# BrandonHanx/TextReID

Measured on AMD Instinct MI355X. Metric: image-text pairs/sec (train), CLIP-RN50 + BiGRU MoCo step, bs128/GPU, higher is better.
Workload: dtype f32; 1 GPU; configs[1]: CLIP-RN50 + GRU, bs128/GPU, 384x128 images, 64-token captions, MoCo queue 8192, fp32, 1xMI355X; random-init weights, synthetic inputs resident in HBM; global_batch=128, parallelism=dp1, optimizer=Adam (fused multi-tensor), step_launch=eager launches, four streams (chosen by the probe over the recorded step)

## Files before the change

include/textreid_hip.h:

```cpp
#ifndef TEXTREID_HIP_H
#define TEXTREID_HIP_H

#include <stdint.h>

#ifdef __cplusplus
extern "C" {
#endif
#if defined(__GNUC__) || defined(__clang__)
#pragma GCC visibility push(default)
#endif

#define TRID_OK 0
#define TRID_E_INVALID (-1)
#define TRID_E_UNSUPPORTED (-2)

#define TRID_VERSION 100

int trid_version(void);
const char* trid_arch(void);
const char* trid_last_error_string(void);

enum {
    TRID_A_KC = 0,
    TRID_A_MC = 1,
// ... 164 lines not shown
                           void* stream);
int trid_bn_bwd_apply_f32(const float* g, const float* y, const float* act, const float* mean,
                          const float* invstd, const float* scale, const float* shift, const float* dgamma,
                          const float* dbeta, int mask_mode, int pooled, int B, int H, int W, int C, float* dy,
                          float* dres, float* amax, void* stream);
int trid_bn_bwd_reduce_bound_f32(const float* g, const float* y, const float* act, const float* mean,
                                 const float* invstd, const float* scale, const float* shift, int mask_mode, int pooled,
                                 int B, int H, int W, int C, float* dgamma, float* dbeta, float* ws, float* bound,
                                 void* stream);
int trid_bn_bwd_reduce_g_f32(const void* g, int g_fmt, const void* y, int y_fmt, const float* act, const float* mean,
                             const float* invstd, const float* scale, const float* shift, int mask_mode,
                             int pooled, int B, int H, int W, int C, float* dgamma, float* dbeta, float* ws,
                             void* stream);
int trid_bn_bwd_apply_p16_f32(const void* g, int g_fmt, const void* y, int y_fmt, const float* act, const float* mean, const float* invstd,
                              const float* scale, const float* shift, const float* dgamma, const float* dbeta,
                              int mask_mode, int pooled, int B, int H, int W, int C, void* dy, int fmt, void* dres,
                              const float* bound, void* stream);

int trid_bn_bwd_dual_reduce_bound_f32(const float* g, const uint64_t* relu_bits, const float* y1, const float* y2, const float* mean1,
                                      const float* invstd1, const float* scale1, const float* mean2, const float* invstd2,
                                      const float* scale2, long long M, int C, float* dgamma1, float* dgamma2, float* dbeta,
                                      float* dbeta2, float* ws, float* bound1, float* bound2, void* stream);
int trid_bn_bwd_dual_apply_p16_f32(const float* g, const uint64_t* relu_bits, const float* y1, const float* y2, const float* mean1,
                                   const float* invstd1, const float* scale1, const float* mean2, const float* invstd2,
                                   const float* scale2, const float* dgamma1, const float* dgamma2, const float* dbeta, long long M,
                                   int C, void* dy1, void* dy2, const float* bound1, const float* bound2, void* stream);

int trid_attnpool_tokens_f32(const float* x, const float* pos, float* tok, int B, int T, int C, int ldt,
                             void* stream);
int trid_attnpool_tokens_fmt_f32(const void* x, int x_fmt, const float* x_amax, const float* pos, float* tok, int B, int T,
                                 int C, int ldt, void* stream);
int trid_attnpool_tokens_bwd_f32(const float* dtok, float* dx, float* dpos, int B, int T, int C, int ldt,
                                 void* stream);
int trid_softmax_rows_f32(float* s, long long rows, int n, int ld, void* stream);
int trid_softmax_rows_bwd_f32(const float* p, const float* dp, float* ds, long long rows, int n, int ld,
                              void* stream);
int trid_colsum_f32(const float* x, float* out, long long M, int N, long long ld, int accumulate, void* stream);

int trid_embedding_gather_f32(const float* table, const int64_t* tokens, float* x, int B, int L, int ldtok, int E,
                              long long vocab, void* stream);
int trid_embedding_bwd_f32(const float* dX, const int64_t* tokens, int B, int L, int ldtok, int E, float* dtable,
                           long long vocab, long long padding_idx, void* stream);
int trid_gru_cell_fwd_f32(const float* gi, const float* gh, float* h, const int64_t* lengths, float* gates,
                          float* hprev, float* maxv, int32_t* argt, int s, int Lmax, int L, int B, int Hd,
                          long long gates_dstride, long long hprev_dstride, void* stream);
int trid_gru_max_init_f32(float* maxv, int32_t* argt, const int64_t* lengths, int Lmax, const int64_t* lmax_dev, int B,
                          int Hd, void* stream);
int trid_gru_cell_bwd_f32(const float* dout, const int32_t* argt, const float* gates, const float* hprev,
                          const int64_t* lengths, float* dh, float* dGi, float* dgh, int s, int Lmax, int L,
                          int B, int Hd, long long gates_dstride, long long hprev_dstride, long long dgh_dstride,
                          void* stream);

long long trid_gru_whh_image_bytes(int H);
int trid_gru_step_workgroups(int B, int H);
int trid_gru_pack_whh_f16(const float* w_hh, const float* w_amax, void* img_fwd, void* img_bwd, int H, void* stream);
int trid_gru_step_fwd_f32(const void* img_fwd, const float* w_amax, const void* hp_in, void* hp_out, float* h,
                          const float* gi, const int64_t* lengths, float* gates, float* hprev, float* maxv,
                          int32_t* argt, int s, int Lmax, int L, int B, int Bp, int H, long long gates_dstride,
                          long long hprev_dstride, void* stream);
int trid_gru_step_bwd_f32(const void* img_bwd, const float* w_amax, const float* dgh_in, const float* amax_in,
                          float* amax_out, const float* dout, const int32_t* argt, const float* gates,
                          const float* hprev, const int64_t* lengths, float* dh, float* dGi, float* dgh_out, int s,
                          int Lmax, int L, int B, int H, long long gates_dstride, long long hprev_dstride,
                          long long dgh_dstride, void* stream);

int trid_gru_step_seq_fwd_f32(const void* img_fwd, const float* w_amax, const void* hp_in, void* hp_out, float* h,
// ... 133 lines not shown
```

textreid_amd/backbones/m_resnet.py:

```python

import logging
import math
import os
from collections import OrderedDict

import torch
from torch import nn

from .. import ops


class Bottleneck(nn.Module):
    expansion = 4

    def __init__(self, inplanes, planes, stride=1):
        super().__init__()
        self.conv1 = nn.Conv2d(inplanes, planes, 1, bias=False)
        self.bn1 = nn.BatchNorm2d(planes)
        self.conv2 = nn.Conv2d(planes, planes, 3, padding=1, bias=False)
        self.bn2 = nn.BatchNorm2d(planes)
        self.avgpool = nn.AvgPool2d(stride) if stride > 1 else nn.Identity()
        self.conv3 = nn.Conv2d(planes, planes * 4, 1, bias=False)
        self.bn3 = nn.BatchNorm2d(planes * 4)
        self.relu = nn.ReLU(inplace=True)
# ... 28 lines not shown
        self.v_proj = nn.Linear(embed_dim, embed_dim)
        self.c_proj = nn.Linear(embed_dim, output_dim or embed_dim)
        self.num_heads = num_heads

    def forward(self, x):
        raise RuntimeError("AttentionPool2d is a parameter holder; call ModifiedResNet.forward")


def _w3x3(conv):
    w = conv.weight
    N, C = w.shape[0], w.shape[1]
    return w.permute(0, 2, 3, 1).contiguous().reshape(N, 9 * C)


def _g3x3(dw, N, C):
    return dw.view(N, 3, 3, C).permute(0, 3, 1, 2)


def _bn_coeffs(bn, partials, M, training, counters=None):
    if training:
        st = ops.bn_finalize(partials, M, bn.weight, bn.bias, bn.running_mean, bn.running_var)
        if counters is None:
            bn.num_batches_tracked += 1
        else:
            counters.append(bn.num_batches_tracked)
        return st
    return ops.bn_eval_coeffs(bn.weight, bn.bias, bn.running_mean, bn.running_var)


import os as _os
_SERIAL_WGRAD = "1" in (_os.environ.get("TRID_SERIAL_WGRAD", "0"), _os.environ.get("TRID_SERIAL", "0"))
_SERIAL_ATTN_WGRAD = _os.environ.get("TRID_SERIAL_ATTN_WGRAD", "0") == "1"
_EARLY_WPT = _os.environ.get("TRID_EARLY_WPT", "1") != "0"
_BATCH_WGRAD = int(_os.environ.get("TRID_WGRAD_BATCH", "1"))


class _WgradStream:

    def __init__(self, device):
        self.main = torch.cuda.current_stream(device)
        self.side = _WgradStream._streams.setdefault(device, torch.cuda.Stream(device=device))
        self.side.wait_stream(self.main)
        self.pending = []
        self.blocks = 0

    _streams = {}

    def run(self, fn, *tensors, keep=()):
        if _SERIAL_WGRAD:
            return fn(*tensors)
        ev = torch.cuda.Event()
        ev.record(self.main)
        self.side.wait_event(ev)
        for t in tensors + tuple(k for k in keep if k is not None):
            t.record_stream(self.side)
        with torch.cuda.stream(self.side):
            out = fn(*tensors)
        out.record_stream(self.main)
        return out

    def defer(self, G, key, fn, tensors, keep=(), post=None):
        if _SERIAL_WGRAD or not _BATCH_WGRAD:
            out = self.run(fn, *tensors, keep=keep)
            G[key] = post(out) if post is not None else out
            return
        self.pending.append((G, key, fn, tensors, keep, post))
# ... 647 lines not shown
            if not stem16:
                x = ops.p16_pack(x, ax, fmt)
            for blk in self.blocks():
                x, rec = block_forward_p16(blk, x, WP, images.device, training, save, nbt, masks)
                if save:
                    S["blocks"].append(rec)
                if taps is not None:
                    taps[names[id(blk)]] = x.unpack()
            if save:
                S["p16"] = fmt
        else:
            for blk in self.blocks():
                x, ax, rec = block_forward(blk, x, ax, ar, training, save, nbt, masks)
                if save:
                    S["blocks"].append(rec)
                if taps is not None:
                    taps[names[id(blk)]] = x
        if nbt:
            torch._foreach_add_(nbt, 1)
        feat, asave = self._attnpool_forward(x, save)
        if save:
            S["attn"] = asave
        return feat, S

    def _attnpool_forward(self, x, save):
        ap = self.attnpool
        B, H, W, C = x.shape
        T = H * W
        T1 = T + 1
        T1p = (T1 + 3) // 4 * 4
        heads = ap.num_heads
        hd = C // heads
        scale = float(hd) ** -0.5
        xd = x.data if isinstance(x, ops.P16) else x
        x_fmt = x.fmt if isinstance(x, ops.P16) else 0
        tok = ops.empty((B, T1p, C), xd)
        ops.call("trid_attnpool_tokens_fmt_f32", ops._p(xd), x_fmt, ops._p(x.amax) if x_fmt == 1 else None, ops._p(ap.positional_embedding),
                 ops._p(tok), B, T, C, T1p, ops.stream())
        x = tok
        q = ops.linear(tok[:, 0], ap.q_proj.weight, ap.q_proj.bias)
        U = ops.empty((B, heads, C), x)
        ops.gemm(q, ap.k_proj.weight, U, B, C, hd, C, C, heads * C, b_mode=ops.B_NC, alpha=scale, batch=heads,
                 strideA=hd, strideB=hd * C, strideC=C)
        P = ops.empty((B, heads, T1p), x)
        ops.gemm(U, tok, P, heads, T1p, C, C, C, T1p, batch=B, strideA=heads * C, strideB=T1p * C, strideC=heads * T1p)
        ops.softmax_rows_(P, T1)
        Z = ops.empty((B, heads, C), x)
        ops.gemm(P, tok, Z, heads, C, T1p, T1p, C, C, b_mode=ops.B_NC, batch=B, strideA=heads * T1p, strideB=T1p * C,
                 strideC=heads * C)
        o = ops.empty((B, C), x)
        ops.gemm(Z, ap.v_proj.weight, o, B, hd, C, heads * C, C, C, batch=heads, strideA=C, strideB=hd * C, strideC=hd,
                 bias=ap.v_proj.bias, strideBias=hd)
        out = ops.linear(o, ap.c_proj.weight, ap.c_proj.bias)
        return out, (((B, H, W, C), tok, q, U, P, Z, o) if save else None)

    def _attnpool_backward(self, asave, gout, G, ws=None):
        ap = self.attnpool
        xshape, tok, q, U, P, Z, o = asave
        B, H, W, C = xshape
        T = H * W
        T1 = T + 1
        T1p = tok.shape[1]
        heads = ap.num_heads
        hd = C // heads
        scale = float(hd) ** -0.5
        Wq, Wk, Wv, Wc = ap.q_proj.weight, ap.k_proj.weight, ap.v_proj.weight, ap.c_proj.weight
        def side(key, fn, *tensors):
            if ws is None or _SERIAL_ATTN_WGRAD:
                G[key] = fn(*tensors)
            else:
                ws.defer(G, key, fn, tensors)

        do = ops.matmul_nn(gout, Wc)
        side(id(Wc), lambda g_, o_: ops.matmul_tn(g_, o_), gout, o)
        side(id(ap.c_proj.bias), lambda g_: ops.colsum(g_), gout)
        side(id(ap.v_proj.bias), lambda d_: ops.colsum(d_), do)

        def dwv(do_, Z_):
            out = torch.empty_like(Wv)
            ops.gemm(do_, Z_, out, hd, C, B, C, heads * C, C, a_mode=ops.A_MC, b_mode=ops.B_NC, batch=heads, strideA=hd,
                     strideB=C, strideC=hd * C)
            return out

        side(id(Wv), dwv, do, Z)
        dZ = ops.empty((B, heads, C), tok)
        ops.gemm(do, Wv, dZ, B, C, hd, C, C, heads * C, b_mode=ops.B_NC, batch=heads, strideA=hd, strideB=hd * C,
                 strideC=C)
        dP = ops.empty((B, heads, T1p), tok)
        ops.gemm(dZ, tok, dP, heads, T1p, C, C, C, T1p, batch=B, strideA=heads * C, strideB=T1p * C,
                 strideC=heads * T1p)
        dS = ops.softmax_rows_bwd(P, dP, T1, out=dP)
        dtok = ops.empty((B, T1p, C), tok)
        ops.gemm(P, dZ, dtok, T1p, C, heads, T1p, C, C, a_mode=ops.A_MC, b_mode=ops.B_NC, batch=B,
                 strideA=heads * T1p, strideB=heads * C, strideC=T1p * C)
        ops.gemm(dS, U, dtok, T1p, C, heads, T1p, C, C, a_mode=ops.A_MC, b_mode=ops.B_NC, batch=B,
                 strideA=heads * T1p, strideB=heads * C, strideC=T1p * C, accumulate=True)
        dU = ops.empty((B, heads, C), tok)
        ops.gemm(dS, tok, dU, heads, C, T1p, T1p, C, C, b_mode=ops.B_NC, batch=B, strideA=heads * T1p,
                 strideB=T1p * C, strideC=heads * C)
        dq = ops.empty((B, C), tok)
        ops.gemm(dU, Wk, dq, B, hd, C, heads * C, C, C, alpha=scale, batch=heads, strideA=C, strideB=hd * C, strideC=hd)
        def dwk(q_, dU_):
            out = torch.empty_like(Wk)
            ops.gemm(q_, dU_, out, hd, C, B, C, heads * C, C, a_mode=ops.A_MC, b_mode=ops.B_NC, alpha=scale, batch=heads,
                     strideA=hd, strideB=C, strideC=hd * C)
            return out

        side(id(Wk), dwk, q, dU)
        G[id(ap.k_proj.bias)] = torch.zeros_like(ap.k_proj.bias)
        ops.matmul_nn(dq, Wq, out=dtok[:, 0], accumulate=True)
        side(id(Wq), lambda dq_, tok_: ops.matmul_tn(dq_, tok_[:, 0]), dq, tok)
        side(id(ap.q_proj.bias), lambda dq_: ops.colsum(dq_), dq)
        dx = ops.empty((B, H, W, C), tok)
        dpos = torch.empty_like(ap.positional_embedding)
        ops.call("trid_attnpool_tokens_bwd_f32", ops._p(dtok), ops._p(dx), ops._p(dpos), B, T, C, T1p, ops.stream())
        G[id(ap.positional_embedding)] = dpos
        if ws is not None:
            ws.flush()
        return dx

    def _run_backward(self, S, gout):
        G = {}
        ws = _WgradStream(gout.device)
        ar = ConvArith(gout.device, S.get("wamax", {}), S.get("prec"))
        g = self._attnpool_backward(S["attn"], gout, G, ws)
        S["attn"] = None
        blocks = list(self.blocks())
        sync = self.grad_sync
        staged = set()

        def stage_ready():
            if sync is None:
                return
            ws.join()
            ps = [p for p in self.parameters() if id(p) in G and id(p) not in staged and G[id(p)] is not None]
            staged.update(id(p) for p in ps)
            sync.stage(ps, [G[id(p)] for p in ps])

        first_of_layer = {id(layer[0]) for layer in (self.layer1, self.layer2, self.layer3, self.layer4)}
        dbg = getattr(self, "_debug_grads", None)
        p16 = S.get("p16", 0)
        WPT = (S.get("WPT") or p16_weights(self, ar.WA, True, p16)) if p16 else None
        if p16 == 2 and ops.BF16_GRADS:
            g = g.to(torch.bfloat16)
        rblocks, rrecs = list(reversed(blocks)), list(reversed(S["blocks"]))
        g_sums = None
        for bi, (blk, rec) in enumerate(zip(rblocks, rrecs)):
            if dbg is not None:
# ... 72 lines not shown
```

textreid_amd/ops.py:

```python

import ctypes
import os
import math

import torch

from . import lib as L
from .lib import GemmDesc, call

A_KC, A_MC, A_CONV = L.TRID_A_KC, L.TRID_A_MC, L.TRID_A_CONV
B_KC, B_NC, B_CONV = L.TRID_B_KC, L.TRID_B_NC, L.TRID_B_CONV

BN_EPS = 1e-5
BN_MOMENTUM = 0.1
STATS_ROWS = 128
GEMM_PRECISION = int(__import__("os").environ.get("TRID_GEMM_PRECISION", "6"))
CONV_PRECISION = int(__import__("os").environ.get("TRID_CONV_PRECISION", "16"))


def conv_precision():
    return CONV_PRECISION if GEMM_PRECISION == 6 else GEMM_PRECISION


_raw_stream = torch._C._cuda_getCurrentRawStream
# ... 1009 lines not shown


def _bn_ws(C, like):
    key = (C, like.device, stream(like.device))
    ws = _ws_cache.get(key)
    if ws is None:
        ws = empty((L.load().trid_bn_bwd_ws_floats(C),), like)
        _ws_cache[key] = ws
    return ws


def bn_bwd(g, y, st, gamma_like, mask_mode, act=None, pooled=False, want_dres=False, amax=None):
    Bi, H, W, C = y.shape
    dg = empty((2, C), y)
    dgamma, dbeta = dg[0], dg[1]
    ws = _bn_ws(C, y)
    call("trid_bn_bwd_reduce_f32", _p(g), _p(y), _p(act), _p(st.mean), _p(st.invstd), _p(st.scale), _p(st.shift),
         mask_mode, 1 if pooled else 0, Bi, H, W, C, _p(dgamma), _p(dbeta), _p(ws), stream())
    dy = torch.empty_like(y)
    dres = torch.empty_like(y) if want_dres else None
    call("trid_bn_bwd_apply_f32", _p(g), _p(y), _p(act), _p(st.mean), _p(st.invstd), _p(st.scale), _p(st.shift),
         _p(dgamma), _p(dbeta), mask_mode, 1 if pooled else 0, Bi, H, W, C, _p(dy), _p(dres), _p(amax), stream())
    return dy, dgamma, dbeta, dres


def colsum(x2d, out=None, accumulate=False):
    M, N = x2d.shape
    if out is None:
        out = empty((N,), x2d)
    call("trid_colsum_f32", _p(x2d), _p(out), M, N, x2d.stride(0), 1 if accumulate else 0, stream())
    return out


def softmax_rows_(s, n):
    rows, ld = s.numel() // s.shape[-1], s.shape[-1]
    call("trid_softmax_rows_f32", _p(s), rows, n, ld, stream())
    return s


def softmax_rows_bwd(p, dp, n, out=None):
    rows, ld = p.numel() // p.shape[-1], p.shape[-1]
    if out is None:
        out = torch.empty_like(p)
    call("trid_softmax_rows_bwd_f32", _p(p), _p(dp), _p(out), rows, n, ld, stream())
    return out


def l2norm_rows(x, eps=1e-12):
    rows, C = x.shape
    y = torch.empty_like(x)
    inv = empty((rows,), x)
    call("trid_l2norm_rows_f32", _p(x), _p(y), _p(inv), rows, C, eps, stream())
    return y, inv


def l2norm_rows_bwd(dy, y, inv, dx=None, accumulate=False):
    rows, C = y.shape
    if dx is None:
        dx = torch.empty_like(y)
    call("trid_l2norm_rows_bwd_f32", _p(dy), _p(y), _p(inv), _p(dx), rows, C, 1 if accumulate else 0, stream())
    return dx


def rowdot(x, y):
    rows, C = x.shape
    out = empty((rows,), x)
# ... 16 lines not shown
```

Measured before the change: 3163 pairs/s.

## Fuse attention-pool token construction into score and weighted-sum kernels

Measured after the change: 3190 pairs/s (median of 6 runs). Within noise of the previous version (+0.8%).

```diff
diff --git a/include/textreid_hip.h b/include/textreid_hip.h
--- a/include/textreid_hip.h
+++ b/include/textreid_hip.h
@@ -220,6 +220,17 @@
                                  int C, int ldt, void* stream);
 int trid_attnpool_tokens_bwd_f32(const float* dtok, float* dx, float* dpos, int B, int T, int C, int ldt,
                                  void* stream);
+int trid_attnpool_fused_ok(int B, int T, int C, int heads, int x_fmt);
+int trid_attnpool_mean_fmt_f32(const void* x, int x_fmt, const float* x_amax, const float* pos, float* tok0, int B, int T,
+                               int C, void* stream);
+int trid_attnpool_scores_fmt_f32(const void* x, int x_fmt, const float* x_amax, const float* tok0, const float* pos,
+                                 const float* A, float* S, int B, int T, int C, int heads, int ldp, void* stream);
+int trid_attnpool_wsum_fmt_f32(const void* x, int x_fmt, const float* x_amax, const float* tok0, const float* pos,
+                               const float* W, float* out, int B, int T, int C, int heads, int ldp, void* stream);
+int trid_attnpool_dtok0_f32(const float* P, const float* dS, const float* dZ, const float* U, float* dtok0, int B, int C,
+                            int heads, int ldp, void* stream);
+int trid_attnpool_dx_f32(const float* P, const float* dS, const float* dZ, const float* U, const float* dtok0, float* dx,
+                         float* dpos, int B, int T, int C, int heads, int ldp, void* stream);
 int trid_softmax_rows_f32(float* s, long long rows, int n, int ld, void* stream);
 int trid_softmax_rows_bwd_f32(const float* p, const float* dp, float* ds, long long rows, int n, int ld,
                               void* stream);
diff --git a/textreid_amd/backbones/m_resnet.py b/textreid_amd/backbones/m_resnet.py
--- a/textreid_amd/backbones/m_resnet.py
+++ b/textreid_amd/backbones/m_resnet.py
@@ -84,6 +84,7 @@
 _SERIAL_WGRAD = "1" in (_os.environ.get("TRID_SERIAL_WGRAD", "0"), _os.environ.get("TRID_SERIAL", "0"))
 _SERIAL_ATTN_WGRAD = _os.environ.get("TRID_SERIAL_ATTN_WGRAD", "0") == "1"
 _EARLY_WPT = _os.environ.get("TRID_EARLY_WPT", "1") != "0"
+_ATTNPOOL_FUSED = _os.environ.get("TRID_ATTNPOOL_FUSED", "1") != "0"
 _BATCH_WGRAD = int(_os.environ.get("TRID_WGRAD_BATCH", "1"))
 
 
@@ -797,35 +798,51 @@
         heads = ap.num_heads
         hd = C // heads
         scale = float(hd) ** -0.5
-        xd = x.data if isinstance(x, ops.P16) else x
-        x_fmt = x.fmt if isinstance(x, ops.P16) else 0
-        tok = ops.empty((B, T1p, C), xd)
-        ops.call("trid_attnpool_tokens_fmt_f32", ops._p(xd), x_fmt, ops._p(x.amax) if x_fmt == 1 else None, ops._p(ap.positional_embedding),
-                 ops._p(tok), B, T, C, T1p, ops.stream())
-        x = tok
-        q = ops.linear(tok[:, 0], ap.q_proj.weight, ap.q_proj.bias)
-        U = ops.empty((B, heads, C), x)
-        ops.gemm(q, ap.k_proj.weight, U, B, C, hd, C, C, heads * C, b_mode=ops.B_NC, alpha=scale, batch=heads,
-                 strideA=hd, strideB=hd * C, strideC=C)
-        P = ops.empty((B, heads, T1p), x)
-        ops.gemm(U, tok, P, heads, T1p, C, C, C, T1p, batch=B, strideA=heads * C, strideB=T1p * C, strideC=heads * T1p)
-        ops.softmax_rows_(P, T1)
-        Z = ops.empty((B, heads, C), x)
-        ops.gemm(P, tok, Z, heads, C, T1p, T1p, C, C, b_mode=ops.B_NC, batch=B, strideA=heads * T1p, strideB=T1p * C,
-                 strideC=heads * C)
+        pos = ap.positional_embedding
+        if _ATTNPOOL_FUSED and ops.attnpool_fused_ok(x, heads):
+            tok0 = ops.attnpool_mean(x, pos)
+            q = ops.linear(tok0, ap.q_proj.weight, ap.q_proj.bias)
+            U = ops.empty((B, heads, C), tok0)
+            ops.gemm(q, ap.k_proj.weight, U, B, C, hd, C, C, heads * C, b_mode=ops.B_NC, alpha=scale, batch=heads,
+                     strideA=hd, strideB=hd * C, strideC=C)
+            P = ops.attnpool_scores(x, tok0, pos, U, ops.empty((B, heads, T1p), tok0))
+            ops.softmax_rows_(P, T1)
+            Z = ops.attnpool_wsum(x, tok0, pos, P)
+            src = (x, tok0)
+            x = tok0
+        else:
+            xd = x.data if isinstance(x, ops.P16) else x
+            x_fmt = x.fmt if isinstance(x, ops.P16) else 0
+            tok = ops.empty((B, T1p, C), xd)
+            ops.call("trid_attnpool_tokens_fmt_f32", ops._p(xd), x_fmt, ops._p(x.amax) if x_fmt == 1 else None, ops._p(pos),
+                     ops._p(tok), B, T, C, T1p, ops.stream())
+            x = tok
+            q = ops.linear(tok[:, 0], ap.q_proj.weight, ap.q_proj.bias)
+            U = ops.empty((B, heads, C), x)
+            ops.gemm(q, ap.k_proj.weight, U, B, C, hd, C, C, heads * C, b_mode=ops.B_NC, alpha=scale, batch=heads,
+                     strideA=hd, strideB=hd * C, strideC=C)
+            P = ops.empty((B, heads, T1p), x)
+            ops.gemm(U, tok, P, heads, T1p, C, C, C, T1p, batch=B, strideA=heads * C, strideB=T1p * C, strideC=heads * T1p)
+            ops.softmax_rows_(P, T1)
+            Z = ops.empty((B, heads, C), x)
+            ops.gemm(P, tok, Z, heads, C, T1p, T1p, C, C, b_mode=ops.B_NC, batch=B, strideA=heads * T1p, strideB=T1p * C,
+                     strideC=heads * C)
+            src = tok
         o = ops.empty((B, C), x)
         ops.gemm(Z, ap.v_proj.weight, o, B, hd, C, heads * C, C, C, batch=heads, strideA=C, strideB=hd * C, strideC=hd,
                  bias=ap.v_proj.bias, strideBias=hd)
         out = ops.linear(o, ap.c_proj.weight, ap.c_proj.bias)
-        return out, (((B, H, W, C), tok, q, U, P, Z, o) if save else None)
+        return out, (((B, H, W, C), src, q, U, P, Z, o) if save else None)
 
     def _attnpool_backward(self, asave, gout, G, ws=None):
         ap = self.attnpool
-        xshape, tok, q, U, P, Z, o = asave
+        xshape, src, q, U, P, Z, o = asave
+        fused = isinstance(src, tuple)
+        tok = src[1] if fused else src
         B, H, W, C = xshape
         T = H * W
         T1 = T + 1
-        T1p = tok.shape[1]
+        T1p = P.shape[2]
         heads = ap.num_heads
         hd = C // heads
         scale = float(hd) ** -0.5
@@ -851,18 +868,24 @@
         dZ = ops.empty((B, heads, C), tok)
         ops.gemm(do, Wv, dZ, B, C, hd, C, C, heads * C, b_mode=ops.B_NC, batch=heads, strideA=hd, strideB=hd * C,
                  strideC=C)
-        dP = ops.empty((B, heads, T1p), tok)
-        ops.gemm(dZ, tok, dP, heads, T1p, C, C, C, T1p, batch=B, strideA=heads * C, strideB=T1p * C,
-                 strideC=heads * T1p)
-        dS = ops.softmax_rows_bwd(P, dP, T1, out=dP)
-        dtok = ops.empty((B, T1p, C), tok)
-        ops.gemm(P, dZ, dtok, T1p, C, heads, T1p, C, C, a_mode=ops.A_MC, b_mode=ops.B_NC, batch=B,
-                 strideA=heads * T1p, strideB=heads * C, strideC=T1p * C)
-        ops.gemm(dS, U, dtok, T1p, C, heads, T1p, C, C, a_mode=ops.A_MC, b_mode=ops.B_NC, batch=B,
-                 strideA=heads * T1p, strideB=heads * C, strideC=T1p * C, accumulate=True)
-        dU = ops.empty((B, heads, C), tok)
-        ops.gemm(dS, tok, dU, heads, C, T1p, T1p, C, C, b_mode=ops.B_NC, batch=B, strideA=heads * T1p,
-                 strideB=T1p * C, strideC=heads * C)
+        pos = ap.positional_embedding
+        if fused:
+            dP = ops.attnpool_scores(src[0], tok, pos, dZ, ops.empty((B, heads, T1p), tok))
+            dS = ops.softmax_rows_bwd(P, dP, T1, out=dP)
+            dU = ops.attnpool_wsum(src[0], tok, pos, dS)
+        else:
+            dP = ops.empty((B, heads, T1p), tok)
+            ops.gemm(dZ, tok, dP, heads, T1p, C, C, C, T1p, batch=B, strideA=heads * C, strideB=T1p * C,
+                     strideC=heads * T1p)
+            dS = ops.softmax_rows_bwd(P, dP, T1, out=dP)
+            dtok = ops.empty((B, T1p, C), tok)
+            ops.gemm(P, dZ, dtok, T1p, C, heads, T1p, C, C, a_mode=ops.A_MC, b_mode=ops.B_NC, batch=B,
+                     strideA=heads * T1p, strideB=heads * C, strideC=T1p * C)
+            ops.gemm(dS, U, dtok, T1p, C, heads, T1p, C, C, a_mode=ops.A_MC, b_mode=ops.B_NC, batch=B,
+                     strideA=heads * T1p, strideB=heads * C, strideC=T1p * C, accumulate=True)
+            dU = ops.empty((B, heads, C), tok)
+            ops.gemm(dS, tok, dU, heads, C, T1p, T1p, C, C, b_mode=ops.B_NC, batch=B, strideA=heads * T1p,
+                     strideB=T1p * C, strideC=heads * C)
         dq = ops.empty((B, C), tok)
         ops.gemm(dU, Wk, dq, B, hd, C, heads * C, C, C, alpha=scale, batch=heads, strideA=C, strideB=hd * C, strideC=hd)
         def dwk(q_, dU_):
@@ -873,12 +896,19 @@
 
         side(id(Wk), dwk, q, dU)
         G[id(ap.k_proj.bias)] = torch.zeros_like(ap.k_proj.bias)
-        ops.matmul_nn(dq, Wq, out=dtok[:, 0], accumulate=True)
-        side(id(Wq), lambda dq_, tok_: ops.matmul_tn(dq_, tok_[:, 0]), dq, tok)
-        side(id(ap.q_proj.bias), lambda dq_: ops.colsum(dq_), dq)
-        dx = ops.empty((B, H, W, C), tok)
-        dpos = torch.empty_like(ap.positional_embedding)
-        ops.call("trid_attnpool_tokens_bwd_f32", ops._p(dtok), ops._p(dx), ops._p(dpos), B, T, C, T1p, ops.stream())
+        dpos = torch.empty_like(pos)
+        if fused:
+            dtok0 = ops.attnpool_dtok0(P, dS, dZ, U)
+            ops.matmul_nn(dq, Wq, out=dtok0, accumulate=True)
+            side(id(Wq), lambda dq_, tok0_: ops.matmul_tn(dq_, tok0_), dq, tok)
+            side(id(ap.q_proj.bias), lambda dq_: ops.colsum(dq_), dq)
+            dx = ops.attnpool_dx(P, dS, dZ, U, dtok0, (B, H, W, C), dpos)
+        else:
+            ops.matmul_nn(dq, Wq, out=dtok[:, 0], accumulate=True)
+            side(id(Wq), lambda dq_, tok_: ops.matmul_tn(dq_, tok_[:, 0]), dq, tok)
+            side(id(ap.q_proj.bias), lambda dq_: ops.colsum(dq_), dq)
+            dx = ops.empty((B, H, W, C), tok)
+            ops.call("trid_attnpool_tokens_bwd_f32", ops._p(dtok), ops._p(dx), ops._p(dpos), B, T, C, T1p, ops.stream())
         G[id(ap.positional_embedding)] = dpos
         if ws is not None:
             ws.flush()
diff --git a/textreid_amd/csrc/attn_pool.hip b/textreid_amd/csrc/attn_pool.hip
--- /dev/null
+++ b/textreid_amd/csrc/attn_pool.hip
@@ -0,0 +1,494 @@
+
+#include "split_common.h"
+
+namespace trid {
+
+typedef float ap16f __attribute__((ext_vector_type(16)));
+
+__device__ __forceinline__ float4 ap_add4(float4 a, float4 b) { return make_float4(a.x + b.x, a.y + b.y, a.z + b.z, a.w + b.w); }
+__device__ __forceinline__ float4 ap_zero4() { return make_float4(0.f, 0.f, 0.f, 0.f); }
+__device__ __forceinline__ int ap_row(int r, int kh) { return (r & 3) + 8 * (r >> 2) + 4 * kh; }
+
+__device__ __forceinline__ void ap_xcd_unit(int id, int inner, int& unit, int& in) {
+    const int per = 8 * inner, grp = id / per, w = id - grp * per;
+    unit = 8 * grp + (w & 7);
+    in = w >> 3;
+}
+static inline unsigned ap_xcd_grid(long long units, int inner) { return (unsigned)((units + 7) / 8 * 8 * inner); }
+
+template <int IFMT>
+__device__ __forceinline__ float4 ap_load_x4(const void* __restrict__ x, long long row, int cq, int CQ, float inv) {
+    if (IFMT == 1) return p16_load4_rc(reinterpret_cast<const uint2*>(x), row, cq, CQ, inv);
+    if (IFMT == 2) return bf16_load4(reinterpret_cast<const uint2*>(x), row * CQ + cq);
+    return reinterpret_cast<const float4*>(x)[row * CQ + cq];
+}
+
+typedef float apf4 __attribute__((ext_vector_type(4)));
+constexpr unsigned AP_OOB = 0x80000000u;
+__device__ __forceinline__ __amdgpu_buffer_rsrc_t ap_rsrc(const void* p, long long bytes) {
+    return __builtin_amdgcn_make_buffer_rsrc((void*)p, 0, (unsigned)bytes, 0x00020000);
+}
+__device__ __forceinline__ float4 ap_bload4(const __amdgpu_buffer_rsrc_t& rs, unsigned off) {
+    const apf4 v = __builtin_bit_cast(apf4, __builtin_amdgcn_raw_buffer_load_b128(rs, off, 0, 0));
+    return make_float4(v.x, v.y, v.z, v.w);
+}
+__device__ __forceinline__ float ap_bload1(const __amdgpu_buffer_rsrc_t& rs, unsigned off) {
+    return __builtin_bit_cast(float, __builtin_amdgcn_raw_buffer_load_b32(rs, off, 0, 0));
+}
+template <int IFMT>
+__device__ __forceinline__ uint4 ap_bload_x4_raw(const __amdgpu_buffer_rsrc_t& rs, unsigned row, int cq, int CQ, bool ok) {
+    if (IFMT == 1) {
+        const unsigned off = ok ? row * (unsigned)CQ * 16u + (unsigned)((cq >> 3) * 16 + (cq & 7)) * 8u : AP_OOB;
+        const uint2 h = __builtin_bit_cast(uint2, __builtin_amdgcn_raw_buffer_load_b64(rs, off, 0, 0));
+        const uint2 l = __builtin_bit_cast(uint2, __builtin_amdgcn_raw_buffer_load_b64(rs, off + 64u, 0, 0));
+        return make_uint4(h.x, h.y, l.x, l.y);
+    }
+    if (IFMT == 2) {
+        const uint2 u = __builtin_bit_cast(uint2, __builtin_amdgcn_raw_buffer_load_b64(rs, ok ? (row * (unsigned)CQ + (unsigned)cq) * 8u : AP_OOB, 0, 0));
+        return make_uint4(u.x, u.y, 0u, 0u);
+    }
+    return __builtin_bit_cast(uint4, __builtin_amdgcn_raw_buffer_load_b128(rs, ok ? (row * (unsigned)CQ + (unsigned)cq) * 16u : AP_OOB, 0, 0));
+}
+template <int IFMT>
+__device__ __forceinline__ float4 ap_decode_x4(uint4 q, float inv) {
+    if (IFMT == 1) {
+        const f16x2 h0 = __builtin_bit_cast(f16x2, q.x), h1 = __builtin_bit_cast(f16x2, q.y);
+        const f16x2 l0 = __builtin_bit_cast(f16x2, q.z), l1 = __builtin_bit_cast(f16x2, q.w);
+        return make_float4(((float)h0.x + (float)l0.x) * inv, ((float)h0.y + (float)l0.y) * inv,
+                           ((float)h1.x + (float)l1.x) * inv, ((float)h1.y + (float)l1.y) * inv);
+    }
+    if (IFMT == 2)
+        return make_float4(__builtin_bit_cast(float, q.x << 16), __builtin_bit_cast(float, q.x & 0xffff0000u),
+                           __builtin_bit_cast(float, q.y << 16), __builtin_bit_cast(float, q.y & 0xffff0000u));
+    return make_float4(__builtin_bit_cast(float, q.x), __builtin_bit_cast(float, q.y), __builtin_bit_cast(float, q.z), __builtin_bit_cast(float, q.w));
+}
+template <int IFMT>
+__device__ __forceinline__ float4 ap_bload_x4(const __amdgpu_buffer_rsrc_t& rs, unsigned row, int cq, int CQ, float inv, bool ok) {
+    return ap_decode_x4<IFMT>(ap_bload_x4_raw<IFMT>(rs, row, cq, CQ, ok), inv);
+}
+__device__ __forceinline__ long long ap_x_bytes(int IFMT, long long rows, int CQ) { return rows * CQ * (IFMT == 2 ? 8 : 16); }
+
+template <int IFMT>
+__global__ __launch_bounds__(256) void attnpool_mean_kernel(const void* __restrict__ x, const float* __restrict__ x_amax,
+                                                            const float4* __restrict__ pos, float4* __restrict__ tok0, int T, int CQ) {
+    __shared__ float4 red[4][64];
+    const int cl = threadIdx.x & 63, tl = threadIdx.x >> 6;
+    const int cq = blockIdx.x * 64 + cl, b = blockIdx.y;
+    const bool live = cq < CQ;
+    const float inv_scale = IFMT == 1 ? 1.f / f16_scale_of(*x_amax) : 1.f;
+    float4 s = ap_zero4();
+    if (live) {
+#pragma unroll 4
+        for (int t = tl; t < T; t += 4) s = ap_add4(s, ap_load_x4<IFMT>(x, (long long)b * T + t, cq, CQ, inv_scale));
+    }
+    red[tl][cl] = s;
+    __syncthreads();
+    if (tl == 0 && live) {
+        const float4 a = red[0][cl], c = red[1][cl], d = red[2][cl], e = red[3][cl];
+        const float inv = 1.f / (float)T;
+        const float4 p0 = pos[cq];
+        tok0[(long long)b * CQ + cq] = make_float4(((a.x + c.x) + (d.x + e.x)) * inv + p0.x, ((a.y + c.y) + (d.y + e.y)) * inv + p0.y,
+                                                  ((a.z + c.z) + (d.z + e.z)) * inv + p0.z, ((a.w + c.w) + (d.w + e.w)) * inv + p0.w);
+    }
+}
+
+constexpr int AP_LD = 132;
+
+template <int IFMT>
+__global__ __launch_bounds__(256) void attnpool_scores_kernel(const void* __restrict__ x, const float* __restrict__ x_amax,
+                                                              const float4* __restrict__ tok0, const float4* __restrict__ pos,
+                                                              const float4* __restrict__ A, float* __restrict__ S, int B, int T,
+                                                              int CQ, int heads, int ldp) {
+    __shared__ float sA[32 * AP_LD];
+    __shared__ float sT[32 * AP_LD];
+    __shared__ float red[4][32][33];
+    const int tid = threadIdx.x, lane = tid & 63, wave = tid >> 6, r = lane & 31, kh = lane >> 5;
+    int b, tile;
+    ap_xcd_unit(blockIdx.x, (T + 31) / 32, b, tile);
+    if (b >= B) return;
+    const int t0 = 1 + tile * 32;
+    const float inv_scale = IFMT == 1 ? 1.f / f16_scale_of(*x_amax) : 1.f;
+    const int lq = tid & 31, lr = tid >> 5;
+    const __amdgpu_buffer_rsrc_t rsX = ap_rsrc(x, ap_x_bytes(IFMT, (long long)B * T, CQ));
+    const __amdgpu_buffer_rsrc_t rsP = ap_rsrc(pos, (long long)(T + 1) * CQ * 16);
+    const __amdgpu_buffer_rsrc_t rsA = ap_rsrc(A, (long long)B * heads * CQ * 16);
+    float4 ra[4], rp[4], rk[4];
+    uint4 rx[4];
+#pragma unroll
+    for (int j = 0; j < 4; ++j) rk[j] = ap_zero4();
+    auto gload = [&](int chunk) {
+        const int cq = chunk * 32 + lq;
+#pragma unroll
+        for (int i = 0; i < 4; ++i) {
+            const int row = lr + 8 * i, t = t0 + row;
+            const bool tok_ok = t <= T;
+            ra[i] = ap_bload4(rsA, row < heads ? (unsigned)((b * heads + row) * CQ + cq) * 16u : AP_OOB);
+            rx[i] = ap_bload_x4_raw<IFMT>(rsX, (unsigned)(b * T + t - 1), cq, CQ, tok_ok);
+            rp[i] = ap_bload4(rsP, tok_ok ? (unsigned)(t * CQ + cq) * 16u : AP_OOB);
+        }
+        if (tile == 0) {
+#pragma unroll
+            for (int j = 0; j < 4; ++j) rk[j] = tok0[(long long)b * CQ + chunk * 32 + 4 * (tid & 7) + j];
+        }
+    };
+    ap16f acc;
+#pragma unroll
+    for (int i = 0; i < 16; ++i) acc[i] = 0.f;
+    float s0 = 0.f;
+    const int nch = CQ / 32;
+    gload(0);
+    for (int ch = 0; ch < nch; ++ch) {
+        __syncthreads();
+#pragma unroll
+        for (int i = 0; i < 4; ++i) {
+            *reinterpret_cast<float4*>(&sA[(lr + 8 * i) * AP_LD + 4 * lq]) = ra[i];
+            *reinterpret_cast<float4*>(&sT[(lr + 8 * i) * AP_LD + 4 * lq]) = ap_add4(ap_decode_x4<IFMT>(rx[i], inv_scale), rp[i]);
+        }
+        __syncthreads();
+        if (tile == 0) {
+            const int h = tid >> 3, part = tid & 7;
+#pragma unroll
+            for (int j = 0; j < 4; ++j) {
+                const float4 u = *reinterpret_cast<const float4*>(&sA[h * AP_LD + 16 * part + 4 * j]);
+                s0 = fmaf(u.w, rk[j].w, fmaf(u.z, rk[j].z, fmaf(u.y, rk[j].y, fmaf(u.x, rk[j].x, s0))));
+            }
+        }
+        if (ch + 1 < nch) gload(ch + 1);
+#pragma unroll
+        for (int g = 0; g < 2; ++g) {
+            const int off = r * AP_LD + 32 * wave + 16 * g + 8 * kh;
+            const float4 a0 = *reinterpret_cast<const float4*>(&sA[off]), a1 = *reinterpret_cast<const float4*>(&sA[off + 4]);
+            const float4 v0 = *reinterpret_cast<const float4*>(&sT[off]), v1 = *reinterpret_cast<const float4*>(&sT[off + 4]);
+            acc = __builtin_amdgcn_mfma_f32_32x32x2f32(a0.x, v0.x, acc, 0, 0, 0);
+            acc = __builtin_amdgcn_mfma_f32_32x32x2f32(a0.y, v0.y, acc, 0, 0, 0);
+            acc = __builtin_amdgcn_mfma_f32_32x32x2f32(a0.z, v0.z, acc, 0, 0, 0);
+            acc = __builtin_amdgcn_mfma_f32_32x32x2f32(a0.w, v0.w, acc, 0, 0, 0);
+            acc = __builtin_amdgcn_mfma_f32_32x32x2f32(a1.x, v1.x, acc, 0, 0, 0);
+            acc = __builtin_amdgcn_mfma_f32_32x32x2f32(a1.y, v1.y, acc, 0, 0, 0);
+            acc = __builtin_amdgcn_mfma_f32_32x32x2f32(a1.z, v1.z, acc, 0, 0, 0);
+            acc = __builtin_amdgcn_mfma_f32_32x32x2f32(a1.w, v1.w, acc, 0, 0, 0);
+        }
+    }
+#pragma unroll
+    for (int i = 0; i < 16; ++i) red[wave][ap_row(i, kh)][r] = acc[i];
+    __syncthreads();
+    for (int idx = tid; idx < 1024; idx += 256) {
+        const int h = idx >> 5, j = idx & 31;
+        const float s = ((red[0][h][j] + red[1][h][j]) + red[2][h][j]) + red[3][h][j];
+        if (h < heads && t0 + j <= T) S[((long long)b * heads + h) * ldp + t0 + j] = s;
+    }
+    if (tile == 0) {
+        s0 += __shfl_xor(s0, 1, 64);
+        s0 += __shfl_xor(s0, 2, 64);
+        s0 += __shfl_xor(s0, 4, 64);
+        if ((tid & 7) == 0 && (tid >> 3) < heads) S[((long long)b * heads + (tid >> 3)) * ldp] = s0;
+    }
+}
+
+struct ApSumFrag {
+    float a[4];
+    float4 v[4];
+};
+
+template <int IFMT>
+__global__ __launch_bounds__(256) void attnpool_wsum_kernel(const void* __restrict__ x, const float* __restrict__ x_amax,
+                                                            const float4* __restrict__ tok0, const float4* __restrict__ pos,
+                                                            const float* __restrict__ Wt, float4* __restrict__ out, int T, int CQ,
+                                                            int heads, int ldp) {
+    __shared__ float smem[3 * 32 * AP_LD];
+    __shared__ float w0[32];
+    float(*red)[32][AP_LD] = reinterpret_cast<float(*)[32][AP_LD]>(smem);
+    const int tid = threadIdx.x, lane = tid & 63, wave = tid >> 6, r = lane & 31, kh = lane >> 5;
+    const int b = blockIdx.y, cq = blockIdx.x * 32 + r;
+    const float inv_scale = IFMT == 1 ? 1.f / f16_scale_of(*x_amax) : 1.f;
+    const __amdgpu_buffer_rsrc_t rsX = ap_rsrc(x, ap_x_bytes(IFMT, (long long)gridDim.y * T, CQ));
+    const __amdgpu_buffer_rsrc_t rsP = ap_rsrc(pos, (long long)(T + 1) * CQ * 16);
+    const int ldw = (T + 1) | 1;
+    {
+        const int n4 = heads * ldp / 4;
+        const __amdgpu_buffer_rsrc_t rsW = ap_rsrc(Wt + (long long)b * heads * ldp, (long long)n4 * 16);
+        for (int base = 0; base < n4; base += 1024) {
+            float4 v[4];
+#pragma unroll
+            for (int k = 0; k < 4; ++k) v[k] = ap_bload4(rsW, base + tid + 256 * k < n4 ? (unsigned)(base + tid + 256 * k) * 16u : AP_OOB);
+#pragma unroll
+            for (int k = 0; k < 4; ++k) {
+                const int f = 4 * (base + tid + 256 * k), h = f / ldp, t = f - h * ldp;
+                if (f < 4 * n4) {
+                    const float e[4] = {v[k].x, v[k].y, v[k].z, v[k].w};
+#pragma unroll
+                    for (int j = 0; j < 4; ++j)
+                        if (t + j <= T) smem[h * ldw + t + j] = e[j];
+                }
+            }
+        }
+        for (int i = heads * ldw + tid; i < 32 * ldw; i += 256) smem[i] = 0.f;
+        if (tid < 32) w0[tid] = tid < heads ? Wt[((long long)b * heads + tid) * ldp] : 0.f;
+    }
+    __syncthreads();
+    const float* Wr = smem + r * ldw;
+    const int npairs = (T + 1) / 2;
+
+    auto load = [&](ApSumFrag& f, int p0) {
+#pragma unroll
+        for (int u = 0; u < 4; ++u) {
+            const int t = 1 + 2 * (p0 + 4 * u) + kh;
+            const bool ok = t <= T;
+            const float w = Wr[ok ? t : T];
+            f.a[u] = ok ? w : 0.f;
+            f.v[u] = ap_add4(ap_bload_x4<IFMT>(rsX, (unsigned)(b * T + t - 1), cq, CQ, inv_scale, ok),
+                             ap_bload4(rsP, ok ? (unsigned)(t * CQ + cq) * 16u : AP_OOB));
+        }
+    };
+    ap16f acc[4];
+#pragma unroll
+    for (int n = 0; n < 4; ++n)
+#pragma unroll
+        for (int i = 0; i < 16; ++i) acc[n][i] = 0.f;
+    auto mma = [&](const ApSumFrag& f) {
+#pragma unroll
+        for (int u = 0; u < 4; ++u) {
+            acc[0] = __builtin_amdgcn_mfma_f32_32x32x2f32(f.a[u], f.v[u].x, acc[0], 0, 0, 0);
+            acc[1] = __builtin_amdgcn_mfma_f32_32x32x2f32(f.a[u], f.v[u].y, acc[1], 0, 0, 0);
+            acc[2] = __builtin_amdgcn_mfma_f32_32x32x2f32(f.a[u], f.v[u].z, acc[2], 0, 0, 0);
+            acc[3] = __builtin_amdgcn_mfma_f32_32x32x2f32(f.a[u], f.v[u].w, acc[3], 0, 0, 0);
+        }
+    };
+    ApSumFrag f0, f1;
+    load(f0, wave);
+    for (int p0 = wave; p0 < npairs; p0 += 32) {
+        load(f1, p0 + 16);
+        mma(f0);
+        load(f0, p0 + 32);
+        mma(f1);
+    }
+    const float4 k0 = tok0[(long long)b * CQ + cq];
+    __syncthreads();
+    if (wave > 0) {
+#pragma unroll
+        for (int i = 0; i < 16; ++i)
+            *reinterpret_cast<float4*>(&red[wave - 1][ap_row(i, kh)][4 * r]) = make_float4(acc[0][i], acc[1][i], acc[2][i], acc[3][i]);
+    }
+    __syncthreads();
+    if (wave == 0) {
+#pragma unroll
+        for (int i = 0; i < 16; ++i) {
+            const int h = ap_row(i, kh);
+            float4 v = make_float4(acc[0][i], acc[1][i], acc[2][i], acc[3][i]);
+            v = ap_add4(v, *reinterpret_cast<const float4*>(&red[0][h][4 * r]));
+            v = ap_add4(v, *reinterpret_cast<const float4*>(&red[1][h][4 * r]));
+            v = ap_add4(v, *reinterpret_cast<const float4*>(&red[2][h][4 * r]));
+            const float w = w0[h];
+            v = make_float4(fmaf(w, k0.x, v.x), fmaf(w, k0.y, v.y), fmaf(w, k0.z, v.z), fmaf(w, k0.w, v.w));
+            if (h < heads) out[((long long)b * heads + h) * CQ + cq] = v;
+        }
+    }
+}
+
+__global__ __launch_bounds__(256) void attnpool_dtok0_kernel(const float* __restrict__ P, const float* __restrict__ dS,
+                                                             const float4* __restrict__ dZ, const float4* __restrict__ U,
+                                                             float4* __restrict__ d0, int CQ, int heads, int ldp) {
+    __shared__ float4 red[4][64];
+    const int cl = threadIdx.x & 63, hl = threadIdx.x >> 6;
+    const int cq = blockIdx.x * 64 + cl;
+    const long long b = blockIdx.y;
+    const bool live = cq < CQ;
+    float4 s = ap_zero4();
+    if (live) {
+#pragma unroll 4
+        for (int h = hl; h < heads; h += 4) {
+            const float p = P[(b * heads + h) * ldp], d = dS[(b * heads + h) * ldp];
+            const float4 z = dZ[(b * heads + h) * CQ + cq], u = U[(b * heads + h) * CQ + cq];
+            s.x = fmaf(d, u.x, fmaf(p, z.x, s.x));
+            s.y = fmaf(d, u.y, fmaf(p, z.y, s.y));
+            s.z = fmaf(d, u.z, fmaf(p, z.z, s.z));
+            s.w = fmaf(d, u.w, fmaf(p, z.w, s.w));
+        }
+    }
+    red[hl][cl] = s;
+    __syncthreads();
+    if (hl == 0 && live) {
+        const float4 a = red[0][cl], c = red[1][cl], d = red[2][cl], e = red[3][cl];
+        d0[b * CQ + cq] = make_float4((a.x + c.x) + (d.x + e.x), (a.y + c.y) + (d.y + e.y), (a.z + c.z) + (d.z + e.z), (a.w + c.w) + (d.w + e.w));
+    }
+}
+
+__global__ __launch_bounds__(256) void attnpool_dx_kernel(const float* __restrict__ P, const float* __restrict__ dS,
+                                                          const float4* __restrict__ dZ, const float4* __restrict__ U,
+                                                          const float4* __restrict__ d0, float4* __restrict__ dx, int B, int T,
+                                                          int CQ, int heads, int ldp) {
+    const int lane = threadIdx.x & 63, wave = threadIdx.x >> 6, r = lane & 31, kh = lane >> 5;
+    const int ncg = (CQ + 127) / 128;
+    int unit, tile;
+    ap_xcd_unit(blockIdx.x, (T + 31) / 32, unit, tile);
+    if (unit >= B * ncg) return;
+    const int cqb = ((unit % ncg) * 4 + wave) * 32;
+    if (cqb >= CQ) return;
+    const int cq = cqb + r;
+    const long long b = unit / ncg;
+    const int t0 = 1 + tile * 32, t = t0 + r;
+    const bool tok_ok = t <= T;
+    const long long nimg = B;
+    const __amdgpu_buffer_rsrc_t rsP = ap_rsrc(P, nimg * heads * ldp * 4), rsD = ap_rsrc(dS, nimg * heads * ldp * 4);
+    const __amdgpu_buffer_rsrc_t rsZ = ap_rsrc(dZ, nimg * heads * CQ * 16), rsU = ap_rsrc(U, nimg * heads * CQ * 16);
+    ap16f acc[4];
+#pragma unroll
+    for (int n = 0; n < 4; ++n)
+#pragma unroll
+        for (int i = 0; i < 16; ++i) acc[n][i] = 0.f;
+    struct Frag {
+        float a1[2], a2[2];
+        float4 zb[2], ub[2];
+    };
+    auto load = [&](Frag& f, int kk) {
+#pragma unroll
+        for (int u = 0; u < 2; ++u) {
+            const int h = 2 * (kk + u) + kh;
+            const bool hok = h < heads;
+            const unsigned row = (unsigned)((int)b * heads + h);
+            const unsigned aoff = (hok && tok_ok) ? (row * (unsigned)ldp + (unsigned)t) * 4u : AP_OOB;
+            const unsigned boff = hok ? (row * (unsigned)CQ + (unsigned)cq) * 16u : AP_OOB;
+            f.a1[u] = ap_bload1(rsP, aoff);
+            f.a2[u] = ap_bload1(rsD, aoff);
+            f.zb[u] = ap_bload4(rsZ, boff);
+            f.ub[u] = ap_bload4(rsU, boff);
+        }
+    };
+    auto mma = [&](const Frag& f) {
+#pragma unroll
+        for (int u = 0; u < 2; ++u) {
+            acc[0] = __builtin_amdgcn_mfma_f32_32x32x2f32(f.a1[u], f.zb[u].x, acc[0], 0, 0, 0);
+            acc[1] = __builtin_amdgcn_mfma_f32_32x32x2f32(f.a1[u], f.zb[u].y, acc[1], 0, 0, 0);
+            acc[2] = __builtin_amdgcn_mfma_f32_32x32x2f32(f.a1[u], f.zb[u].z, acc[2], 0, 0, 0);
+            acc[3] = __builtin_amdgcn_mfma_f32_32x32x2f32(f.a1[u], f.zb[u].w, acc[3], 0, 0, 0);
+            acc[0] = __builtin_amdgcn_mfma_f32_32x32x2f32(f.a2[u], f.ub[u].x, acc[0], 0, 0, 0);
+            acc[1] = __builtin_amdgcn_mfma_f32_32x32x2f32(f.a2[u], f.ub[u].y, acc[1], 0, 0, 0);
+            acc[2] = __builtin_amdgcn_mfma_f32_32x32x2f32(f.a2[u], f.ub[u].z, acc[2], 0, 0, 0);
+            acc[3] = __builtin_amdgcn_mfma_f32_32x32x2f32(f.a2[u], f.ub[u].w, acc[3], 0, 0, 0);
+        }
+    };
+    const int steps = (heads + 1) / 2;
+    Frag f0, f1;
+    load(f0, 0);
+    for (int kk = 0; kk < steps; kk += 4) {
+        load(f1, kk + 2);
+        mma(f0);
+        load(f0, kk + 4);
+        mma(f1);
+    }
+    const float inv = 1.f / (float)T;
+    const float4 m = d0[b * CQ + cq];
+#pragma unroll
+    for (int i = 0; i < 16; ++i) {
+        const int tt = t0 + ap_row(i, kh);
+        if (tt <= T)
+            dx[(b * T + tt - 1) * CQ + cq] = make_float4(acc[0][i] + m.x * inv, acc[1][i] + m.y * inv, acc[2][i] + m.z * inv, acc[3][i] + m.w * inv);
+    }
+}
+
+__global__ __launch_bounds__(256) void attnpool_dpos0_kernel(const float4* __restrict__ d0, float4* __restrict__ dpos, int B, int CQ) {
+    __shared__ float4 red[16][16];
+    const int cl = threadIdx.x & 15, bl = threadIdx.x >> 4;
+    const int cq = blockIdx.x * 16 + cl;
+    float4 s = ap_zero4();
+    if (cq < CQ) {
+#pragma unroll 8
+        for (int b = bl; b < B; b += 16) s = ap_add4(s, d0[(long long)b * CQ + cq]);
+    }
+    red[bl][cl] = s;
+    __syncthreads();
+    if (bl == 0 && cq < CQ) {
+        for (int k = 1; k < 16; ++k) s = ap_add4(s, red[k][cl]);
+        dpos[cq] = s;
+    }
+}
+
+__global__ __launch_bounds__(256) void attnpool_dpos_kernel(const float4* __restrict__ dx, float4* __restrict__ dpos, int B, int T,
+                                                            int CQ) {
+    __shared__ float4 red[4][64];
+    const int cl = threadIdx.x & 63, bl = threadIdx.x >> 6;
+    const long long col = (long long)blockIdx.x * 64 + cl, ncol = (long long)T * CQ;
+    const bool live = col < ncol;
+    float4 s = ap_zero4();
+    if (live) {
+#pragma unroll 4
+        for (int b = bl; b < B; b += 4) s = ap_add4(s, dx[(long long)b * ncol + col]);
+    }
+    red[bl][cl] = s;
+    __syncthreads();
+    if (bl == 0 && live) {
+        const float4 a = red[0][cl], c = red[1][cl], d = red[2][cl], e = red[3][cl];
+        const float inv = 1.f / (float)T;
+        const float4 m = dpos[col % CQ];
+        dpos[CQ + col] = make_float4(((a.x + c.x) + (d.x + e.x)) - m.x * inv, ((a.y + c.y) + (d.y + e.y)) - m.y * inv,
+                                     ((a.z + c.z) + (d.z + e.z)) - m.z * inv, ((a.w + c.w) + (d.w + e.w)) - m.w * inv);
+    }
+}
+
+static bool attnpool_fused_shape_ok(long long B, long long T, long long C, long long heads, int x_fmt) {
+    return B >= 1 && B <= 65535 && T >= 1 && T <= 3 * AP_LD - 2 && B * (T + 4 > 32 ? T + 4 : 32) * C * 4 < (1ll << 31) && C >= 128 && C % 128 == 0 && C <= (1 << 16) && heads >= 1 && heads <= 32 &&
+           x_fmt >= 0 && x_fmt <= 2;
+}
+
+}
+
+using namespace trid;
+
+#define AP_DISPATCH(kernel, grid, ...)                                                                             \
+    do {                                                                                                           \
+        if (x_fmt == 1) hipLaunchKernelGGL(kernel<1>, grid, dim3(256), 0, (hipStream_t)stream, __VA_ARGS__);       \
+        else if (x_fmt == 2) hipLaunchKernelGGL(kernel<2>, grid, dim3(256), 0, (hipStream_t)stream, __VA_ARGS__);  \
+        else hipLaunchKernelGGL(kernel<0>, grid, dim3(256), 0, (hipStream_t)stream, __VA_ARGS__);                  \
+    } while (0)
+
+extern "C" int trid_attnpool_fused_ok(int B, int T, int C, int heads, int x_fmt) {
+    return attnpool_fused_shape_ok(B, T, C, heads, x_fmt) ? 1 : 0;
+}
+
+extern "C" int trid_attnpool_mean_fmt_f32(const void* x, int x_fmt, const float* x_amax, const float* pos, float* tok0, int B, int T,
+                                          int C, void* stream) {
+    TRID_REQUIRE(x && pos && tok0 && (x_fmt != 1 || x_amax) && attnpool_fused_shape_ok(B, T, C, 1, x_fmt), "trid_attnpool_mean_fmt_f32: bad arguments");
+    const int CQ = C / 4;
+    AP_DISPATCH(attnpool_mean_kernel, dim3((unsigned)((CQ + 63) / 64), (unsigned)B), x, x_amax, (const float4*)pos, (float4*)tok0, T, CQ);
+    return check_launch("trid_attnpool_mean_fmt_f32");
+}
+
+extern "C" int trid_attnpool_scores_fmt_f32(const void* x, int x_fmt, const float* x_amax, const float* tok0, const float* pos,
+                                            const float* A, float* S, int B, int T, int C, int heads, int ldp, void* stream) {
+    TRID_REQUIRE(x && tok0 && pos && A && S && (x_fmt != 1 || x_amax) && ldp >= T + 1 && attnpool_fused_shape_ok(B, T, C, heads, x_fmt),
+                 "trid_attnpool_scores_fmt_f32: bad arguments");
+    AP_DISPATCH(attnpool_scores_kernel, dim3(ap_xcd_grid(B, (T + 31) / 32)), x, x_amax, (const float4*)tok0, (const float4*)pos,
+                (const float4*)A, S, B, T, C / 4, heads, ldp);
+    return check_launch("trid_attnpool_scores_fmt_f32");
+}
+
+extern "C" int trid_attnpool_wsum_fmt_f32(const void* x, int x_fmt, const float* x_amax, const float* tok0, const float* pos,
+                                          const float* W, float* out, int B, int T, int C, int heads, int ldp, void* stream) {
+    TRID_REQUIRE(x && tok0 && pos && W && out && (x_fmt != 1 || x_amax) && ldp >= T + 1 && ldp % 4 == 0 && attnpool_fused_shape_ok(B, T, C, heads, x_fmt),
+                 "trid_attnpool_wsum_fmt_f32: bad arguments (ldp: a multiple of 4)");
+    AP_DISPATCH(attnpool_wsum_kernel, dim3((unsigned)(C / 128), (unsigned)B), x, x_amax, (const float4*)tok0, (const float4*)pos, W,
+                (float4*)out, T, C / 4, heads, ldp);
+    return check_launch("trid_attnpool_wsum_fmt_f32");
+}
+
+extern "C" int trid_attnpool_dtok0_f32(const float* P, const float* dS, const float* dZ, const float* U, float* dtok0, int B, int C,
+                                       int heads, int ldp, void* stream) {
+    TRID_REQUIRE(P && dS && dZ && U && dtok0 && ldp >= 1 && attnpool_fused_shape_ok(B, 1, C, heads, 0), "trid_attnpool_dtok0_f32: bad arguments");
+    hipLaunchKernelGGL(attnpool_dtok0_kernel, dim3((unsigned)((C / 4 + 63) / 64), (unsigned)B), dim3(256), 0, (hipStream_t)stream, P, dS,
+                       (const float4*)dZ, (const float4*)U, (float4*)dtok0, C / 4, heads, ldp);
+    return check_launch("trid_attnpool_dtok0_f32");
+}
+
+extern "C" int trid_attnpool_dx_f32(const float* P, const float* dS, const float* dZ, const float* U, const float* dtok0, float* dx,
+                                    float* dpos, int B, int T, int C, int heads, int ldp, void* stream) {
+    TRID_REQUIRE(P && dS && dZ && U && dtok0 && dx && dpos && ldp >= T + 1 && attnpool_fused_shape_ok(B, T, C, heads, 0),
+                 "trid_attnpool_dx_f32: bad arguments");
+    const int CQ = C / 4;
+    hipStream_t s = (hipStream_t)stream;
+    hipLaunchKernelGGL(attnpool_dx_kernel, dim3(ap_xcd_grid((long long)B * ((CQ + 127) / 128), (T + 31) / 32)), dim3(256), 0, s, P, dS,
+                       (const float4*)dZ, (const float4*)U, (const float4*)dtok0, (float4*)dx, B, T, CQ, heads, ldp);
+    hipLaunchKernelGGL(attnpool_dpos0_kernel, dim3((unsigned)((CQ + 15) / 16)), dim3(256), 0, s, (const float4*)dtok0, (float4*)dpos, B, CQ);
+    const long long ncol = (long long)T * CQ;
+    hipLaunchKernelGGL(attnpool_dpos_kernel, dim3((unsigned)((ncol + 63) / 64)), dim3(256), 0, s, (const float4*)dx, (float4*)dpos, B, T, CQ);
+    return check_launch("trid_attnpool_dx_f32");
+}
diff --git a/textreid_amd/ops.py b/textreid_amd/ops.py
--- a/textreid_amd/ops.py
+++ b/textreid_amd/ops.py
@@ -1065,6 +1065,55 @@
     return out
 
 
+def _x_fmt(x):
+    if isinstance(x, P16):
+        return x.data, x.fmt, (_p(x.amax) if x.fmt == 1 else None)
+    return x, 0, None
+
+
+def attnpool_fused_ok(x, heads):
+    xd, fmt, _ = _x_fmt(x)
+    B, H, W, C = xd.shape
+    return L.load().trid_attnpool_fused_ok(B, H * W, C, heads, fmt) == 1
+
+
+def attnpool_mean(x, pos):
+    xd, fmt, am = _x_fmt(x)
+    B, H, W, C = xd.shape
+    tok0 = empty((B, C), xd)
+    call("trid_attnpool_mean_fmt_f32", _p(xd), fmt, am, _p(pos), _p(tok0), B, H * W, C, stream())
+    return tok0
+
+
+def attnpool_scores(x, tok0, pos, a, out):
+    xd, fmt, am = _x_fmt(x)
+    B, H, W, C = xd.shape
+    call("trid_attnpool_scores_fmt_f32", _p(xd), fmt, am, _p(tok0), _p(pos), _p(a), _p(out), B, H * W, C, a.shape[1], out.shape[2], stream())
+    return out
+
+
+def attnpool_wsum(x, tok0, pos, w):
+    xd, fmt, am = _x_fmt(x)
+    B, H, W, C = xd.shape
+    out = empty((B, w.shape[1], C), xd)
+    call("trid_attnpool_wsum_fmt_f32", _p(xd), fmt, am, _p(tok0), _p(pos), _p(w), _p(out), B, H * W, C, w.shape[1], w.shape[2], stream())
+    return out
+
+
+def attnpool_dtok0(P, dS, dZ, U):
+    B, heads, C = dZ.shape
+    out = empty((B, C), dZ)
+    call("trid_attnpool_dtok0_f32", _p(P), _p(dS), _p(dZ), _p(U), _p(out), B, C, heads, P.shape[2], stream())
+    return out
+
+
+def attnpool_dx(P, dS, dZ, U, dtok0, xshape, dpos):
+    B, H, W, C = xshape
+    dx = empty((B, H, W, C), dZ)
+    call("trid_attnpool_dx_f32", _p(P), _p(dS), _p(dZ), _p(U), _p(dtok0), _p(dx), _p(dpos), B, H * W, C, dZ.shape[1], P.shape[2], stream())
+    return dx
+
+
 def softmax_rows_(s, n):
     rows, ld = s.numel() // s.shape[-1], s.shape[-1]
     call("trid_softmax_rows_f32", _p(s), rows, n, ld, stream())
```
